# Zhongxu-Wang/ArtSpeech

Measured on AMD Instinct MI355X. Metric: mel frames/sec (whole job; per-GPU = value / n_gpus), acoustic-model inference path, batch 32 x 200-frame utterances, higher is better.
Workload: dtype f32 (f16x3 split-operand MFMA, fp32 accumulate)

## Files before the change

### artspeech_amd/csrc/common.h

```cpp
#pragma once
#include <hip/hip_runtime.h>
#include <stdint.h>

#define AS_OK 0
#define AS_EINVAL (-1)
#ifndef AS_EDEVICE
#define AS_EDEVICE (-3)
#endif

unsigned* as_status_words_device();
int as_status_peek();

#define AS_CHECK_LAUNCH()                        \
    do {                                         \
        hipError_t e__ = hipGetLastError();      \
        if (e__ != hipSuccess) return (int)e__;  \
    } while (0)

#define AS_CHECK(call)                           \
    do {                                         \
        hipError_t e__ = (call);                 \
        if (e__ != hipSuccess) return (int)e__;  \
    } while (0)

// ... 21 lines not shown
        if (r__ != AS_OK) return r__;                                              \
    } while (0)

#define AS_WAVE 64

struct AsDynGeo {
    const int32_t* frame_off;
    int32_t B, cap1, n_seg;
    int32_t seg_first[17];
    int32_t seg_cap[16];
    int32_t* seg_frame_off[16];
    int32_t* w[4];
    int32_t* off[4];
    unsigned long long* meta[4];
    int32_t* nvalid[4];
    int32_t* src3;
    int32_t* tof;
    unsigned* status;
};
int as_dyn_geometry_launch(const AsDynGeo& g, hipStream_t stream);
struct AsSegScatter {
    const float* src; int32_t ld_src, rows, n_seg;
    const int32_t* frame_off;
    int32_t seg_first[17];
    int32_t seg_cap[16];
    float* dst[16]; int32_t ld_dst[16];
};
int as_seg_scatter_launch(const AsSegScatter& a, hipStream_t stream);
int as_voice_gather_launch(const float* voices, int ld_voice, int n_voices, const int32_t* idx, int B, int n_style, int n_dur, float* style,
                           int ld_style, float* ds, int ld_ds, hipStream_t stream);
int as_durations_prosody_launch(const float* dur_f32, const int32_t* forced_dur, const int32_t* tok_off, int B, const float* pros, int ld_pros,
                                int32_t* dur_i32, int32_t* frame_off, int32_t* tok_of_frame, int max_frames, hipStream_t stream);
int as_project_cols_prosody_launch(const float* x, int ldx, int K, int N, const float* w, const float* bias, int M, float* y, int ldy,
                                   const float* pros, int ld_pros, const int32_t* col_off, int B, int track0, hipStream_t s);
int as_token_dur_scale_launch(const float* dur_f32, const float* rows, int ld, const int32_t* tok_off, int B, int ntok, const float* pros,
                              int ld_pros, float* out, hipStream_t stream);
int as_token_starts_launch(const int32_t* dur_i32, int ntok, int32_t* start, hipStream_t stream);
int as_token_tracks_launch(float* fne, int ld, int n_cols, const int32_t* tof, int n_frames_max, const int32_t* frame_off, const int32_t* tok_off,
                           int B, int ntok, const int32_t* start, const float* rows, int ld_rows, int smooth, hipStream_t stream);

int as_pcm16_launch(const float* w, int N, const int32_t* n_valid, float* w_fill, int16_t* pcm, hipStream_t stream);

#define AS_VOC_MAX_RATES 9
struct AsVocGeo {
    const int32_t* off;
    int32_t B, mult, cap, max_len, n_rates;
    int32_t rate[AS_VOC_MAX_RATES];
    long long meta_start[AS_VOC_MAX_RATES];
    int32_t* tab;
    unsigned long long* meta;
    int32_t* sample_off;
    unsigned* status;
};
int as_vocoder_cap_geometry_launch(const AsVocGeo& g, hipStream_t stream);

enum { AS_CLS_GEMM = 0, AS_CLS_ADAIN = 1, AS_CLS_LN = 2, AS_CLS_ATTN = 3, AS_CLS_LSTM = 4, AS_CLS_MAS = 5, AS_CLS_OTHER = 6, AS_N_CLS = 7 };
struct AsProfScope {
    int idx;
    hipStream_t stream;
    AsProfScope(int cls, double flops, double bytes, hipStream_t s, const char* tag = nullptr);
    ~AsProfScope();
};

#ifdef __HIPCC__
static __device__ __forceinline__ void as_status_raise(unsigned* words, int kind)
{
    if (words) __hip_atomic_store(words + kind, 1u, __ATOMIC_RELAXED, __HIP_MEMORY_SCOPE_SYSTEM);
}
static __device__ __forceinline__ int as_pcm16(float w, bool* nan)
{
    *nan = w != w;
    return *nan ? 0 : (int)fmaxf(-32768.f, fminf(32767.f, rintf(__fmul_rn(32767.f, w))));
}
static __device__ __forceinline__ float as_adain_val(float x, float mean, float rstd, float one_plus_gamma, float beta, int lrelu)
{
    const float o = __fmaf_rn(one_plus_gamma, __fmul_rn(__fsub_rn(x, mean), rstd), beta);
    return (lrelu && o < 0.f) ? __fmul_rn(0.2f, o) : o;
}
static __device__ __forceinline__ void as_convt_pair(float a0, float a1, float w0, float w1, float w2, float pb, float* o0, float* o1)
{
    *o0 = __fmaf_rn(a0, w1, pb);
    *o1 = __fadd_rn(__fmaf_rn(a1, w0, __fmul_rn(a0, w2)), pb);
}
#endif
```

### artspeech_amd/csrc/conv_gemm_h3.hip

```cpp
#include "conv_gemm.h"
#include <cstring>
#include <type_traits>

typedef __attribute__((address_space(3))) void lds_void;

template <int I, int N, typename F>
static __device__ __forceinline__ void h3_for(F&& f)
{
    if constexpr (I < N) {
        f(std::integral_constant<int, I>{});
        h3_for<I + 1, N>(f);
    }
}

template <int WM, int WN, int WK, int KT, int NS, int NP, int TM = 2>
struct H3Cfg {
    static constexpr int QP = NP == 1 ? 2 : 4;
    static constexpr int BM = 32 * TM * WM, BN = 64 * WN;
    static constexpr int KBS = WK * KT;
    static constexpr int A_BLK = QP * BM * 16, B_BLK = QP * BN * 16;
    static constexpr int A_ST = KBS * A_BLK;
    static constexpr int STAGE = KBS * (A_BLK + B_BLK);
    static constexpr int RED = (WK - 1) * WM * WN * 32 * TM * 64 * 4;
    static constexpr int LDS = NS * STAGE > RED ? NS * STAGE : RED;
// ... 407 lines not shown
{
    if ((double)K * ldx * 4.0 >= 2147483648.0) return AS_EINVAL;
    hipLaunchKernelGGL(split_f16x2_kernel, dim3(as_cdiv(N + 1, 1024), 2 * as_kbx(K)), dim3(256), 0, stream, x, ldx, K, N, n_valid, lrelu, slope,
                       reinterpret_cast<u32x4_t*>(xh));
    AS_CHECK_LAUNCH();
    return AS_OK;
}

extern "C" int as_split_f16x2_f32(const float* x, int ldx, int K, int N, int in_act, float in_slope, uint16_t* xh, as_stream_t stream)
{
    return as_split_f16x2_cap_f32(x, ldx, K, N, nullptr, in_act, in_slope, xh, stream);
}

extern "C" int as_split_f16x2_cap_f32(const float* x, int ldx, int K, int N, const int32_t* n_valid, int in_act, float in_slope, uint16_t* xh,
                                      as_stream_t stream)
{
    if (!x || !xh || K <= 0 || N < 0 || ldx < N || (in_act != 0 && in_act != 2) || !(fabsf(in_slope) <= 3.0e38f)) return AS_EINVAL;
    if ((reinterpret_cast<uintptr_t>(xh) & 15) != 0) return AS_EINVAL;
    if (N == 0) return AS_OK;
    AsProfScope prof__(AS_CLS_OTHER, 0, 8.0 * K * (double)N, (hipStream_t)stream);
    return as_split_f16x2_launch(x, ldx, K, N, in_act == 2, in_slope, xh, (hipStream_t)stream, n_valid);
}

extern "C" size_t as_prep_weight_f16x2_sc_bytes(int G, int Cout, int Cin, int T, int Cin2)
{
    if (G <= 0 || Cout <= 0 || Cin <= 0 || T <= 0 || Cin2 < 0) return 0;
    return (size_t)G * ((size_t)T * as_kbx(Cin) + (Cin2 ? as_kbx(Cin2) : 0)) * 4 * (size_t)Cout * 16;
}
extern "C" size_t as_prep_weight_f16x2_bytes(int G, int Cout, int Cin, int T) { return as_prep_weight_f16x2_sc_bytes(G, Cout, Cin, T, 0); }

extern "C" int as_prep_weight_f16x2_sc_host(const float* w, const float* w2, int G, int Cout, int Cin, int T, int Cin2, uint16_t* wh,
                                            float* scale_out)
{
    if (!w || !wh || !scale_out || G <= 0 || Cout <= 0 || Cin <= 0 || T <= 0 || Cin2 < 0 || ((Cin2 > 0) != (w2 != nullptr))) return AS_EINVAL;
    const size_t n = (size_t)G * Cout * Cin * T, n2 = (size_t)G * Cout * Cin2;
    float mx = 0.f;
    for (size_t i = 0; i < n + n2; ++i) {
        const float x = i < n ? w[i] : w2[i - n];
        const float v = x < 0 ? -x : x;
        if (!(v <= 3.0e38f)) return AS_EINVAL;
        mx = v > mx ? v : mx;
    }
    int e = 0;
    float scale = 1.0f;
    if (mx > 0.f) {
        frexpf(mx, &e);
        scale = ldexpf(1.0f, 14 - e);
    }
    const int KBx = as_kbx(Cin), KBx2 = Cin2 ? as_kbx(Cin2) : 0;
    const size_t blocks = (size_t)T * KBx + KBx2;
    const size_t total = as_prep_weight_f16x2_sc_bytes(G, Cout, Cin, T, Cin2) / 2;
    for (size_t i = 0; i < total; ++i) wh[i] = 0;
    auto put = [&](size_t block, int k, int m, float x) {
        const _Float16 h = (_Float16)x;
        const _Float16 l = (_Float16)(x - (float)h);
        const int kh = (k >> 3) & 1, e8 = k & 7;
        const size_t base = block * 4 * (size_t)Cout * 8;
        uint16_t hb, lb;
        __builtin_memcpy(&hb, &h, 2);
        __builtin_memcpy(&lb, &l, 2);
        wh[base + ((size_t)(0 * 2 + kh) * Cout + m) * 8 + e8] = hb;
        wh[base + ((size_t)(1 * 2 + kh) * Cout + m) * 8 + e8] = lb;
    };
    for (int g = 0; g < G; ++g)
        for (int m = 0; m < Cout; ++m) {
            for (int k = 0; k < Cin; ++k)
                for (int t = 0; t < T; ++t) put((size_t)g * blocks + (size_t)t * KBx + (k >> 4), k, m, w[(((size_t)g * Cout + m) * Cin + k) * T + t] * scale);
            for (int k = 0; k < Cin2; ++k) put((size_t)g * blocks + (size_t)T * KBx + (k >> 4), k, m, w2[((size_t)g * Cout + m) * Cin2 + k] * scale);
        }
    *scale_out = scale;
    return AS_OK;
}
extern "C" int as_prep_weight_f16x2_host(const float* w, int G, int Cout, int Cin, int T, uint16_t* wh, float* scale_out)
{
    return as_prep_weight_f16x2_sc_host(w, nullptr, G, Cout, Cin, T, 0, wh, scale_out);
}

static __device__ __forceinline__ float h3_wave_sum(float v)
{
#pragma unroll
    for (int o = 32; o > 0; o >>= 1) v += __shfl_xor(v, o);
    return v;
}

template <bool UP>
__global__ void __launch_bounds__(256)
adain_image_kernel(const AsAdainArgs a)
{
    const int lane = threadIdx.x & 63, wave = __builtin_amdgcn_readfirstlane(threadIdx.x >> 6);
    const int kb = blockIdx.x * 2 + (wave >> 1), kh = wave & 1, u = blockIdx.y;
    const int C = a.C;
    if (kb >= as_kbx(C)) return;
    const size_t NX = (size_t)a.N + 1;
    u32x4_t* xs = reinterpret_cast<u32x4_t*>(a.yh);
    const size_t plane = ((size_t)kb * 4 + kh) * NX;
    if (u == 0 && lane == 0) {
        xs[plane + a.N] = u32x4_t{0u, 0u, 0u, 0u};
        xs[plane + 2 * NX + a.N] = u32x4_t{0u, 0u, 0u, 0u};
    }
    const int o0 = a.col_off[u], L = a.col_w ? a.col_w[u] : a.col_off[u + 1] - o0;
    if (L <= 0) return;
    const int s0 = a.src_off ? a.src_off[u] : o0;
    const size_t gbase = a.gb_off ? (size_t)a.gb_off[u] : (size_t)u * a.ldgb;
    const int c0 = kb * 16 + kh * 8;
    float g1[8], bt[8], w0[8], w1[8], w2[8], pb[8];
#pragma unroll
    for (int r = 0; r < 8; ++r) {
        const int c = c0 + r < C ? c0 + r : C - 1;
        g1[r] = 1.0f + a.gb[gbase + (size_t)c * a.gb_sc];
        bt[r] = a.gb[gbase + (size_t)(C + c) * a.gb_sc];
        if (UP) { w0[r] = a.pool_w[c * 3 + 0]; w1[r] = a.pool_w[c * 3 + 1]; w2[r] = a.pool_w[c * 3 + 2]; pb[r] = a.pool_b[c]; }
    }
    const float* xr0 = a.x + s0;
    const size_t at0 = plane + (UP ? 2 * (size_t)o0 : (size_t)o0);
    float mean[8], rstd[8];
    auto resident = [&](auto rv_) {
        constexpr int RV = decltype(rv_)::value;
        float v[8][RV];
#pragma unroll
        for (int r = 0; r < 8; ++r) {
            const float* xr = xr0 + (size_t)(c0 + r < C ? c0 + r : C - 1) * a.ldx;
#pragma unroll
            for (int j = 0; j < RV; ++j) v[r][j] = xr[min(lane + 64 * j, L - 1)];
        }
#pragma unroll
        for (int r = 0; r < 8; ++r) {
            float sacc = 0.f;
#pragma unroll
            for (int j = 0; j < RV; ++j)
                if (lane + 64 * j < L) sacc += v[r][j];
            mean[r] = h3_wave_sum(sacc) / (float)L;
        }
#pragma unroll
        for (int r = 0; r < 8; ++r) {
            float vacc = 0.f;
#pragma unroll
            for (int j = 0; j < RV; ++j)
                if (lane + 64 * j < L) { const float d = __fsub_rn(v[r][j], mean[r]); vacc = __fmaf_rn(d, d, vacc); }
            rstd[r] = 1.0f / sqrtf(h3_wave_sum(vacc) / (float)L + 1e-5f);
        }
        if (UP && a.x_up) {
#pragma unroll
            for (int r = 0; r < 8; ++r) {
                if (c0 + r >= C) continue;
                float* ur = a.x_up + (size_t)(c0 + r) * a.ld_up + 2 * o0;
#pragma unroll
                for (int j = 0; j < RV; ++j) {
                    const int i = lane + 64 * j;
                    if (i < L) { ur[2 * i] = v[r][j]; ur[2 * i + 1] = v[r][j]; }
                }
            }
        }
#pragma unroll
        for (int r = 0; r < 8; ++r)
#pragma unroll
            for (int j = 0; j < RV; ++j)
                v[r][j] = (c0 + r < C && lane + 64 * j < L) ? as_adain_val(v[r][j], mean[r], rstd[r], g1[r], bt[r], a.lrelu) : 0.f;
#pragma unroll
        for (int j = 0; j < RV; ++j) {
            const int i = lane + 64 * j;
            if (64 * j >= L) break;
            if (!UP) {
                float t[8];
#pragma unroll
                for (int r = 0; r < 8; ++r) t[r] = v[r][j];
                u32x4_t h, l;
                split2(t, h, l);
                if (i < L) {
                    xs[at0 + i] = h;
                    xs[at0 + i + 2 * NX] = l;
                }
            } else {
                float e0[8], e1[8];
#pragma unroll
                for (int r = 0; r < 8; ++r) {
                    const float dn = __shfl_down(v[r][j], 1);
                    const float wr = j + 1 < RV ? __shfl(v[r][j + 1 < RV ? j + 1 : j], 0) : 0.f;
                    const float an = i + 1 < L ? (lane == 63 ? wr : dn) : 0.f;
                    float o0v, o1v;
                    as_convt_pair(v[r][j], an, w0[r], w1[r], w2[r], pb[r], &o0v, &o1v);
                    e0[r] = c0 + r < C ? o0v : 0.f;
                    e1[r] = c0 + r < C ? o1v : 0.f;
                }
                u32x4_t h, l, h2, l2;
                split2(e0, h, l);
                split2(e1, h2, l2);
                if (i < L) {
                    xs[at0 + 2 * i] = h;
                    xs[at0 + 2 * i + 2 * NX] = l;
                    xs[at0 + 2 * i + 1] = h2;
                    xs[at0 + 2 * i + 1 + 2 * NX] = l2;
                }
            }
        }
    };
    if (L <= 256) { resident(std::integral_constant<int, 4>{}); return; }
    if (L <= 512) { resident(std::integral_constant<int, 8>{}); return; }
    {
        size_t rowoff[8];
#pragma unroll
        for (int r = 0; r < 8; ++r) rowoff[r] = (size_t)(c0 + r < C ? c0 + r : C - 1) * a.ldx;
        float acc[8];
#pragma unroll
        for (int r = 0; r < 8; ++r) acc[r] = 0.f;
        int i = lane;
        for (; i + 192 < L; i += 256) {
            float t[4][8];
#pragma unroll
            for (int q = 0; q < 4; ++q)
#pragma unroll
                for (int r = 0; r < 8; ++r) t[q][r] = xr0[rowoff[r] + i + 64 * q];
#pragma unroll
            for (int q = 0; q < 4; ++q)
#pragma unroll
                for (int r = 0; r < 8; ++r) acc[r] += t[q][r];
        }
        for (; i < L; i += 64)
#pragma unroll
            for (int r = 0; r < 8; ++r) acc[r] += xr0[rowoff[r] + i];
#pragma unroll
        for (int r = 0; r < 8; ++r) { mean[r] = h3_wave_sum(acc[r]) / (float)L; acc[r] = 0.f; }
        i = lane;
        for (; i + 192 < L; i += 256) {
            float t[4][8];
#pragma unroll
            for (int q = 0; q < 4; ++q)
#pragma unroll
                for (int r = 0; r < 8; ++r) t[q][r] = xr0[rowoff[r] + i + 64 * q];
#pragma unroll
            for (int q = 0; q < 4; ++q)
#pragma unroll
                for (int r = 0; r < 8; ++r) { const float d = __fsub_rn(t[q][r], mean[r]); acc[r] = __fmaf_rn(d, d, acc[r]); }
        }
        for (; i < L; i += 64)
#pragma unroll
            for (int r = 0; r < 8; ++r) { const float d = __fsub_rn(xr0[rowoff[r] + i], mean[r]); acc[r] = __fmaf_rn(d, d, acc[r]); }
#pragma unroll
        for (int r = 0; r < 8; ++r) rstd[r] = 1.0f / sqrtf(h3_wave_sum(acc[r]) / (float)L + 1e-5f);
    }
    for (int i0 = lane; i0 < L; i0 += 128) {
        float xi[2][8], xn[2][8];
#pragma unroll
        for (int q = 0; q < 2; ++q) {
            const int i = min(i0 + 64 * q, L - 1);
#pragma unroll
            for (int r = 0; r < 8; ++r) {
                const float* xr = xr0 + (size_t)(c0 + r < C ? c0 + r : C - 1) * a.ldx;
                xi[q][r] = xr[i];
                if (UP) xn[q][r] = xr[min(i + 1, L - 1)];
            }
        }
#pragma unroll
        for (int q = 0; q < 2; ++q) {
            const int i = i0 + 64 * q;
            if (i >= L) break;
            float a0[8], a1[8];
#pragma unroll
            for (int r = 0; r < 8; ++r) {
                const bool ok = c0 + r < C;
                a0[r] = ok ? as_adain_val(xi[q][r], mean[r], rstd[r], g1[r], bt[r], a.lrelu) : 0.f;
                a1[r] = (UP && ok && i + 1 < L) ? as_adain_val(xn[q][r], mean[r], rstd[r], g1[r], bt[r], a.lrelu) : 0.f;
                if (UP && a.x_up && ok) {
                    float* ur = a.x_up + (size_t)(c0 + r) * a.ld_up + 2 * o0 + 2 * i;
                    ur[0] = xi[q][r];
                    ur[1] = xi[q][r];
                }
            }
            u32x4_t h, l;
            if (!UP) {
                split2(a0, h, l);
                xs[at0 + i] = h;
                xs[at0 + i + 2 * NX] = l;
            } else {
                float e0[8], e1[8];
#pragma unroll
                for (int r = 0; r < 8; ++r) {
                    as_convt_pair(a0[r], a1[r], w0[r], w1[r], w2[r], pb[r], &e0[r], &e1[r]);
                    if (c0 + r >= C) { e0[r] = 0.f; e1[r] = 0.f; }
                }
                split2(e0, h, l);
                xs[at0 + 2 * i] = h;
                xs[at0 + 2 * i + 2 * NX] = l;
                split2(e1, h, l);
                xs[at0 + 2 * i + 1] = h;
                xs[at0 + 2 * i + 1 + 2 * NX] = l;
            }
        }
    }
}

extern "C" int as_adain_image_f32(const AsAdainArgs* args_host, as_stream_t stream)
{
    if (!args_host) return AS_EINVAL;
    const AsAdainArgs& a = *args_host;
    if (!a.x || !a.gb || !a.col_off || !a.yh || a.C <= 0 || a.U <= 0 || a.N < 0 || a.gb_sc <= 0 || (!a.gb_off && a.ldgb <= 0)) return AS_EINVAL;
    if ((a.pool_w == nullptr) != (a.pool_b == nullptr) || (a.x_up && !a.pool_w)) return AS_EINVAL;
    if ((reinterpret_cast<uintptr_t>(a.yh) & 15) != 0) return AS_EINVAL;
    if (a.N == 0) return AS_OK;
    AsProfScope prof__(AS_CLS_ADAIN, 0, 8.0 * a.C * (double)a.N, (hipStream_t)stream);
    if (a.pool_w) hipLaunchKernelGGL(adain_image_kernel<true>, dim3(as_kbx(a.C) / 2, a.U), dim3(256), 0, (hipStream_t)stream, a);
    else hipLaunchKernelGGL(adain_image_kernel<false>, dim3(as_kbx(a.C) / 2, a.U), dim3(256), 0, (hipStream_t)stream, a);
    AS_CHECK_LAUNCH();
    return AS_OK;
}

extern "C" int as_adain_split_f32(const float* x, int ldx, int C, const float* gamma_beta, int ldgb, const int32_t* col_off, int B,
                                  int N, int lrelu, uint16_t* xs, as_stream_t stream)
{
    if (!x || !gamma_beta || !col_off || !xs || C <= 0 || B <= 0 || N < 0 || ldgb < 2 * C) return AS_EINVAL;
    AsAdainArgs a = {};
    a.x = x; a.ldx = ldx; a.C = C; a.gb = gamma_beta; a.ldgb = ldgb; a.gb_sc = 1; a.col_off = col_off; a.U = B; a.N = N; a.lrelu = lrelu; a.yh = xs;
    return as_adain_image_f32(&a, stream);
}

__global__ void __launch_bounds__(256)
rows_image_kernel(const float* __restrict__ x, int ldx, int K, int B, u32x4_t* __restrict__ xh)
{
    const int i = blockIdx.x * 256 + threadIdx.x;
    const int groups = 2 * as_kbx(K);
    if (i >= groups * (B + 1)) return;
    const int g = i / (B + 1), b = i % (B + 1);
    float t[8];
#pragma unroll
    for (int r = 0; r < 8; ++r) t[r] = (b < B && g * 8 + r < K) ? x[(size_t)b * ldx + g * 8 + r] : 0.f;
    u32x4_t h, l;
    split2(t, h, l);
    const size_t at = ((size_t)(g >> 1) * 4 + (g & 1)) * (B + 1) + b;
    xh[at] = h;
    xh[at + 2 * (size_t)(B + 1)] = l;
}

extern "C" int as_rows_image_f32(const float* x, int ldx, int K, int B, uint16_t* xh, as_stream_t stream)
{
    if (!x || !xh || K <= 0 || B <= 0 || ldx < K || (reinterpret_cast<uintptr_t>(xh) & 15) != 0) return AS_EINVAL;
    AsProfScope prof__(AS_CLS_OTHER, 0, 8.0 * K * (double)B, (hipStream_t)stream);
    hipLaunchKernelGGL(rows_image_kernel, dim3(as_cdiv((long)2 * as_kbx(K) * (B + 1), 256)), dim3(256), 0, (hipStream_t)stream, x, ldx, K, B,
                       reinterpret_cast<u32x4_t*>(xh));
    AS_CHECK_LAUNCH();
    return AS_OK;
}

#define LNS_COLS 32
#define LNS_PARTS 32
#define LNS_MAXG 4
__global__ void __launch_bounds__(1024)
channel_ln_split_kernel(const float* __restrict__ x, int ldx, int C, int N, const float* __restrict__ gamma1,
                        const float* __restrict__ beta1, const float* __restrict__ gamma2, const float* __restrict__ beta2, int n_split,
                        float eps, int relu, u32x4_t* __restrict__ xs, int KBx)
{
    __shared__ float red[LNS_PARTS][LNS_COLS + 1];
    const int col = threadIdx.x % LNS_COLS, part = threadIdx.x / LNS_COLS;
    const int j = blockIdx.x * LNS_COLS + col;
    const bool ok = j < N;
    const int grp = gamma2 ? j / n_split : 0;
    const float* gamma = gamma1 + (ptrdiff_t)grp * (gamma2 - gamma1);
    const float* beta = beta1 + (ptrdiff_t)grp * (beta2 - beta1);
    const int ngroups = 2 * KBx;
    float v[LNS_MAXG][8];
    float s = 0.f;
#pragma unroll
    for (int i = 0; i < LNS_MAXG; ++i)
#pragma unroll
        for (int r = 0; r < 8; ++r) {
            const int c = 8 * (part + i * LNS_PARTS) + r;
            v[i][r] = (ok && c < C) ? x[(size_t)c * ldx + j] : 0.f;
            s += v[i][r];
        }
    red[part][col] = s;
    __syncthreads();
    float tot = 0.f;
#pragma unroll
    for (int q = 0; q < LNS_PARTS; ++q) tot += red[q][col];
    const float mean = tot / (float)C;
    __syncthreads();
    float q2 = 0.f;
#pragma unroll
    for (int i = 0; i < LNS_MAXG; ++i)
#pragma unroll
        for (int r = 0; r < 8; ++r) {
            const int c = 8 * (part + i * LNS_PARTS) + r;
            const float d = __fsub_rn(v[i][r], mean);
            if (c < C) q2 = __fmaf_rn(d, d, q2);
        }
    red[part][col] = q2;
    __syncthreads();
    tot = 0.f;
#pragma unroll
    for (int q = 0; q < LNS_PARTS; ++q) tot += red[q][col];
    const float rs = 1.0f / sqrtf(tot / (float)C + eps);
    const size_t NX = (size_t)N + 1;
    if (blockIdx.x == 0 && col == 0) {
#pragma unroll
        for (int i = 0; i < LNS_MAXG; ++i) {
            const int g = part + i * LNS_PARTS;
            if (g < ngroups)
                for (int p = 0; p < 2; ++p) xs[((size_t)(g >> 1) * 4 + (g & 1) + 2 * p) * NX + N] = u32x4_t{0u, 0u, 0u, 0u};
        }
    }
    if (!ok) return;
#pragma unroll
    for (int i = 0; i < LNS_MAXG; ++i) {
        const int g = part + i * LNS_PARTS;
        if (g >= ngroups) continue;
        float t[8];
#pragma unroll
        for (int r = 0; r < 8; ++r) {
            const int c = 8 * g + r;
            float o = 0.f;
            if (c < C) {
                o = __fmaf_rn(__fmul_rn(__fsub_rn(v[i][r], mean), rs), gamma[c], beta[c]);
                if (relu) o = o < 0.f ? 0.f : o;
            }
            t[r] = o;
        }
        u32x4_t h, l;
        split2(t, h, l);
        const size_t at = ((size_t)(g >> 1) * 4 + (g & 1)) * NX + j;
        xs[at] = h;
        xs[at + 2 * NX] = l;
    }
}

extern "C" int as_channel_layernorm_split_f32(const float* x, int ldx, int C, int N, const float* gamma, const float* beta,
                                              const float* gamma2, const float* beta2, int n_split, float eps, int relu, uint16_t* xs,
                                              as_stream_t stream)
{
    if (!x || !xs || !gamma || !beta || C <= 0 || C > 8 * LNS_PARTS * LNS_MAXG || N <= 0 || ldx < N ||
        ((gamma2 == nullptr) != (beta2 == nullptr)) || (gamma2 && n_split <= 0) || (reinterpret_cast<uintptr_t>(xs) & 15) != 0)
        return AS_EINVAL;
    const int KBx = as_kbx(C);
    AsProfScope prof__(AS_CLS_LN, 8.0 * C * N, 8.0 * C * (double)N, (hipStream_t)stream);
    hipLaunchKernelGGL(channel_ln_split_kernel, dim3(as_cdiv(N, LNS_COLS)), dim3(1024), 0, (hipStream_t)stream, x, ldx, C, N, gamma, beta,
                       gamma2, beta2, n_split, eps, relu, reinterpret_cast<u32x4_t*>(xs), KBx);
    AS_CHECK_LAUNCH();
    return AS_OK;
}
```

### artspeech_amd/csrc/elementwise.hip

```cpp
#include "common.h"
#include <algorithm>
#include <cstring>
#include "artspeech_hip.h"
#include "conv_gemm.h"
#include "down_strips.h"
#include <cstdint>
#include <type_traits>
#define AS_FILE_CLS AS_CLS_OTHER

static __device__ __forceinline__ float wave_sum(float v)
{
#pragma unroll
    for (int o = 32; o > 0; o >>= 1) v += __shfl_xor(v, o);
    return v;
}

static __device__ __forceinline__ float lrelu02(float v) { return v > 0.f ? v : 0.2f * v; }

__global__ void make_meta_kernel(const int* __restrict__ widths, const int* __restrict__ col_off, int B, int H,
                                 unsigned long long* __restrict__ meta, unsigned* __restrict__ status)
{
    const int b = blockIdx.y;
    const int W = widths[b];
    const int base = col_off[b];
// ... 136 lines not shown

extern "C" int as_channel_layernorm_f32(const float* x, int ldx, int C, int N, const float* gamma, const float* beta,
                                        float eps, int relu, float* y, int ldy, as_stream_t stream)
{
    return as_channel_layernorm_groups_f32(x, ldx, C, N, gamma, beta, nullptr, nullptr, 0, eps, relu, y, ldy, stream);
}

__global__ void __launch_bounds__(256)
adain_kernel(const float* __restrict__ x, int ldx, int C, const float* __restrict__ gb, int ldgb,
             const int* __restrict__ col_off, int B, float* __restrict__ y, int ldy, int act,
             const float* __restrict__ pool_w, const float* __restrict__ pool_b, float* __restrict__ xup, int ldup)
{
    const int lane = threadIdx.x & 63;
    const int row = blockIdx.x * 4 + (threadIdx.x >> 6);
    if (row >= C * B) return;
    const int c = row / B, b = row - c * B;
    const int o0 = col_off[b], L = col_off[b + 1] - o0;
    if (L <= 0) return;
    const float* xr = x + (size_t)c * ldx + o0;
    float s = 0.f;
    for (int i = lane; i < L; i += 64) s += xr[i];
    const float mean = wave_sum(s) / (float)L;
    float v = 0.f;
    for (int i = lane; i < L; i += 64) { const float d = __fsub_rn(xr[i], mean); v = __fmaf_rn(d, d, v); }
    const float var = wave_sum(v) / (float)L;
    const float rs = 1.0f / sqrtf(var + 1e-5f);
    const float g = 1.0f + gb[(size_t)b * ldgb + c];
    const float be = gb[(size_t)b * ldgb + C + c];
    if (!pool_w) {
        float* yr = y + (size_t)c * ldy + o0;
        for (int i = lane; i < L; i += 64) yr[i] = as_adain_val(xr[i], mean, rs, g, be, act);
    } else {
        const float w0 = pool_w[c * 3 + 0], w1 = pool_w[c * 3 + 1], w2 = pool_w[c * 3 + 2], pb = pool_b[c];
        float* yr = y + (size_t)c * ldy + 2 * o0;
        float* ur = xup ? xup + (size_t)c * ldup + 2 * o0 : nullptr;
        for (int i = lane; i < L; i += 64) {
            const float xi = xr[i];
            const float a0 = as_adain_val(xi, mean, rs, g, be, act);
            const float a1 = i + 1 < L ? as_adain_val(xr[i + 1], mean, rs, g, be, act) : 0.f;
            float e0, e1;
            as_convt_pair(a0, a1, w0, w1, w2, pb, &e0, &e1);
            yr[2 * i] = e0;
            yr[2 * i + 1] = e1;
            if (ur) { ur[2 * i] = xi; ur[2 * i + 1] = xi; }
        }
    }
}

extern "C" int as_adain_f32(const float* x, int ldx, int C, const float* gamma_beta, int ldgb, const int32_t* col_off,
                            int B, float* y, int ldy, int lrelu, const float* pool_w, const float* pool_b,
                            float* x_up, int ld_up, as_stream_t stream)
{
    if (!x || !y || !gamma_beta || !col_off || C <= 0 || B < 0 || ldgb < 2 * C) return AS_EINVAL;
    if ((pool_w == nullptr) != (pool_b == nullptr)) return AS_EINVAL;
    if (B == 0) return AS_OK;
    AsProfScope prof__(AS_CLS_ADAIN, 0, 0, (hipStream_t)stream);
    hipLaunchKernelGGL(adain_kernel, dim3(as_cdiv((long)C * B, 4)), dim3(256), 0, (hipStream_t)stream, x, ldx, C,
                       gamma_beta, ldgb, col_off, B, y, ldy, lrelu, pool_w, pool_b, x_up, ld_up);
    AS_CHECK_LAUNCH();
    return AS_OK;
}

template <int KR>
__global__ void __launch_bounds__(256)
linear_rows_kernel(const float* __restrict__ x, int ldx, const float* __restrict__ w, const float* __restrict__ bias,
                   int B, int M, int K, float* __restrict__ y, int ldy)
{
    static_assert(KR == 1 || KR == 2 || KR == 4 || KR == 8, "quads of the weight row per lane");
    const int lane = threadIdx.x & 63;
    const int m = blockIdx.x * 4 + (threadIdx.x >> 6);
    if (m >= M) return;
    const float* wr = w + (size_t)m * K;
    const float bm = bias ? bias[m] : 0.f;
    const bool vec = (K & 3) == 0 && (ldx & 3) == 0 && ((reinterpret_cast<uintptr_t>(w) | reinterpret_cast<uintptr_t>(x)) & 15) == 0;
    if (vec && K <= 256 * KR) {
        constexpr int RT = 32 / KR;
        const int nq = K >> 2;
        float4 wq[KR];
#pragma unroll
        for (int c = 0; c < KR; ++c) {
            const int q = lane + 64 * c;
            wq[c] = q < nq ? reinterpret_cast<const float4*>(wr)[q] : make_float4(0.f, 0.f, 0.f, 0.f);
        }
        for (int b0 = 0; b0 < B; b0 += RT) {
            float4 v[RT][KR];
#pragma unroll
            for (int r = 0; r < RT; ++r) {
                const float4* xq = reinterpret_cast<const float4*>(x + (size_t)min(b0 + r, B - 1) * ldx);
#pragma unroll
                for (int c = 0; c < KR; ++c) {
                    const int q = lane + 64 * c;
                    v[r][c] = xq[q < nq ? q : 0];
                }
            }
#pragma unroll
            for (int r = 0; r < RT; ++r) {
                float s = 0.f;
#pragma unroll
                for (int c = 0; c < KR; ++c) s += wq[c].x * v[r][c].x + wq[c].y * v[r][c].y + wq[c].z * v[r][c].z + wq[c].w * v[r][c].w;
                s = wave_sum(s);
                if (lane == 0 && b0 + r < B) y[(size_t)(b0 + r) * ldy + m] = s + bm;
            }
        }
        return;
    }
    for (int b = 0; b < B; ++b) {
        const float* xr = x + (size_t)b * ldx;
        float s = 0.f;
        for (int k = lane; k < K; k += 64) s += wr[k] * xr[k];
        s = wave_sum(s);
        if (lane == 0) y[(size_t)b * ldy + m] = s + bm;
    }
}

extern "C" int as_linear_rows_f32(const float* x, int ldx, const float* w, const float* bias, int B, int M, int K,
                                  float* y, int ldy, as_stream_t stream)
{
    if (!x || !w || !y || B < 0 || M <= 0 || K <= 0 || ldx < K || ldy < M) return AS_EINVAL;
    if (B == 0) return AS_OK;
    AsProfScope prof__(AS_FILE_CLS, 0, 0, (hipStream_t)stream);
    const dim3 grid(as_cdiv(M, 4)), block(256);
    hipStream_t s_ = (hipStream_t)stream;
    if (K <= 256) hipLaunchKernelGGL(linear_rows_kernel<1>, grid, block, 0, s_, x, ldx, w, bias, B, M, K, y, ldy);
    else if (K <= 512) hipLaunchKernelGGL(linear_rows_kernel<2>, grid, block, 0, s_, x, ldx, w, bias, B, M, K, y, ldy);
    else if (K <= 1024) hipLaunchKernelGGL(linear_rows_kernel<4>, grid, block, 0, s_, x, ldx, w, bias, B, M, K, y, ldy);
    else hipLaunchKernelGGL(linear_rows_kernel<8>, grid, block, 0, s_, x, ldx, w, bias, B, M, K, y, ldy);
    AS_CHECK_LAUNCH();
    return AS_OK;
}

template <int MM>
__global__ void __launch_bounds__(256)
project_cols_kernel(const float* __restrict__ x, int ldx, int K, int N, const float* w, const float* __restrict__ bias, int M,
                    float* __restrict__ y, int ldy, const float* __restrict__ pros, int ldr, const int* __restrict__ col_off, int B, int track0)
{
    __shared__ float part[3][MM][64];
    extern __shared__ __attribute__((aligned(16))) float wsm[];
    for (int i = threadIdx.x; i < MM * K; i += 256) {
        const int k = i / MM, m = i % MM;
        wsm[i] = m < M ? w[(size_t)m * K + k] : 0.f;
    }
    __syncthreads();
    w = wsm;
    const int lane = threadIdx.x & 63, wave = threadIdx.x >> 6;
    const int j = blockIdx.x * 64 + lane;
    const bool ok = j < N;
    float acc[MM];
#pragma unroll
    for (int m = 0; m < MM; ++m) acc[m] = 0.f;
    int k = wave;
    const float* xc = x + (ok ? j : 0);
    for (; k + 60 < K; k += 64) {
        float v[16];
#pragma unroll
        for (int u = 0; u < 16; ++u) v[u] = xc[(size_t)(k + 4 * u) * ldx];
#pragma unroll
        for (int u = 0; u < 16; ++u)
#pragma unroll
            for (int m = 0; m < MM; ++m)
                acc[m] += w[(k + 4 * u) * MM + m] * v[u];
    }
    for (; k + 12 < K; k += 16) {
        float v[4];
#pragma unroll
        for (int u = 0; u < 4; ++u) v[u] = xc[(size_t)(k + 4 * u) * ldx];
#pragma unroll
        for (int u = 0; u < 4; ++u)
#pragma unroll
            for (int m = 0; m < MM; ++m)
                acc[m] += w[(k + 4 * u) * MM + m] * v[u];
    }
    for (; k < K; k += 4) {
        const float v = xc[(size_t)k * ldx];
#pragma unroll
        for (int m = 0; m < MM; ++m)
            acc[m] += w[k * MM + m] * v;
    }
    if (wave > 0) {
#pragma unroll
        for (int m = 0; m < MM; ++m) part[wave - 1][m][lane] = acc[m];
    }
    __syncthreads();
    if (wave != 0 || !ok) return;
    const float* r = nullptr;
    if (pros) {
        int lo = 0, hi = B;
        while (hi > lo) {
            const int mid = (lo + hi + 1) >> 1;
            if (col_off[mid] <= j) lo = mid;
            else hi = mid - 1;
        }
        if (lo < B) r = pros + (size_t)lo * ldr + track0;
    }
#pragma unroll
    for (int m = 0; m < MM; ++m) {
        if (m >= M) continue;
        const float v = ((acc[m] + part[0][m][lane]) + (part[1][m][lane] + part[2][m][lane])) + (bias ? bias[m] : 0.f);
        y[(size_t)m * ldy + j] = r ? __builtin_fmaf(r[AS_PROSODY_GAIN + m], v, r[AS_PROSODY_OFFSET + m]) : v;
    }
}

extern "C" int as_project_cols_f32(const float* x, int ldx, int K, int N, const float* w, const float* bias, int M, float* y, int ldy,
                                   as_stream_t stream)
{
// ... 1043 lines not shown
```

Measured before the change: 1.785 million.

## Batch wave reductions and vectorize loads in AdaIN, channel LN and linear-rows kernels

Adds an 8-way batched wave reduction built on ds_bpermute and uses it in the AdaIN image kernel and the linear-rows kernel, so independent per-row sums share one LDS wait per step instead of each running its own shuffle chain. AdaIN now loads its per-utterance offsets with one lane-parallel load and broadcasts them with readlane, gathers gamma/beta/pool weights across lanes, and writes upsample pairs as float2. Channel LN is templated on the group count so registers and loops match C, and it loads the affine parameters early with float4 reads. Linear-rows gets a second grid dimension over batch rows so small-M launches fill more of the GPU. The inline asm and the wider templating add register pressure and code-size risk.

```diff
diff --git a/artspeech_amd/csrc/common.h b/artspeech_amd/csrc/common.h
--- a/artspeech_amd/csrc/common.h
+++ b/artspeech_amd/csrc/common.h
@@ -127,4 +127,25 @@
     *o0 = __fmaf_rn(a0, w1, pb);
     *o1 = __fadd_rn(__fmaf_rn(a1, w0, __fmul_rn(a0, w2)), pb);
 }
+static __device__ __forceinline__ void as_wave_sum8(float (&s)[8])
+{
+    const int lane = __lane_id();
+#pragma unroll
+    for (int o = 32; o > 0; o >>= 1) {
+        const int at = (lane ^ o) << 2;
+        float t0, t1, t2, t3, t4, t5, t6, t7;
+        asm volatile("ds_bpermute_b32 %0, %8, %9\n\t"
+                     "ds_bpermute_b32 %1, %8, %10\n\t"
+                     "ds_bpermute_b32 %2, %8, %11\n\t"
+                     "ds_bpermute_b32 %3, %8, %12\n\t"
+                     "ds_bpermute_b32 %4, %8, %13\n\t"
+                     "ds_bpermute_b32 %5, %8, %14\n\t"
+                     "ds_bpermute_b32 %6, %8, %15\n\t"
+                     "ds_bpermute_b32 %7, %8, %16\n\t"
+                     "s_waitcnt lgkmcnt(0)"
+                     : "=&v"(t0), "=&v"(t1), "=&v"(t2), "=&v"(t3), "=&v"(t4), "=&v"(t5), "=&v"(t6), "=&v"(t7)
+                     : "v"(at), "v"(s[0]), "v"(s[1]), "v"(s[2]), "v"(s[3]), "v"(s[4]), "v"(s[5]), "v"(s[6]), "v"(s[7]));
+        s[0] += t0; s[1] += t1; s[2] += t2; s[3] += t3; s[4] += t4; s[5] += t5; s[6] += t6; s[7] += t7;
+    }
+}
 #endif
diff --git a/artspeech_amd/csrc/conv_gemm_h3.hip b/artspeech_amd/csrc/conv_gemm_h3.hip
--- a/artspeech_amd/csrc/conv_gemm_h3.hip
+++ b/artspeech_amd/csrc/conv_gemm_h3.hip
@@ -513,7 +513,6 @@
     for (int o = 32; o > 0; o >>= 1) v += __shfl_xor(v, o);
     return v;
 }
-
 template <bool UP>
 __global__ void __launch_bounds__(256)
 adain_image_kernel(const AsAdainArgs a)
@@ -522,28 +521,65 @@
     const int kb = blockIdx.x * 2 + (wave >> 1), kh = wave & 1, u = blockIdx.y;
     const int C = a.C;
     if (kb >= as_kbx(C)) return;
+    const int32_t* __restrict__ col_off = a.col_off;
+    const int32_t* __restrict__ col_w = a.col_w;
+    const int32_t* __restrict__ src_off = a.src_off;
+    const int32_t* __restrict__ gb_off = a.gb_off;
+    const float* __restrict__ gb = a.gb;
+    const float* __restrict__ pool_w = a.pool_w;
+    const float* __restrict__ pool_b = a.pool_b;
+    int word = 0;
+    {
+        const int32_t* p = col_off + u;
+        if (lane == 1 && !col_w) p = col_off + u + 1;
+        if (lane == 2 && col_w) p = col_w + u;
+        if (lane == 3 && src_off) p = src_off + u;
+        if (lane == 4 && gb_off) p = gb_off + u;
+        if (lane < 5) word = *p;
+    }
+    const int o0 = __builtin_amdgcn_readlane(word, 0);
+    const int L = col_w ? __builtin_amdgcn_readlane(word, 2) : __builtin_amdgcn_readlane(word, 1) - o0;
+    const int s0 = src_off ? __builtin_amdgcn_readlane(word, 3) : o0;
+    const size_t gbase = gb_off ? (size_t)__builtin_amdgcn_readlane(word, 4) : (size_t)u * a.ldgb;
     const size_t NX = (size_t)a.N + 1;
     u32x4_t* xs = reinterpret_cast<u32x4_t*>(a.yh);
     const size_t plane = ((size_t)kb * 4 + kh) * NX;
-    if (u == 0 && lane == 0) {
-        xs[plane + a.N] = u32x4_t{0u, 0u, 0u, 0u};
-        xs[plane + 2 * NX + a.N] = u32x4_t{0u, 0u, 0u, 0u};
-    }
-    const int o0 = a.col_off[u], L = a.col_w ? a.col_w[u] : a.col_off[u + 1] - o0;
-    if (L <= 0) return;
-    const int s0 = a.src_off ? a.src_off[u] : o0;
-    const size_t gbase = a.gb_off ? (size_t)a.gb_off[u] : (size_t)u * a.ldgb;
+    auto zero_column = [&]() {
+        if (u == 0 && lane == 0) {
+            xs[plane + a.N] = u32x4_t{0u, 0u, 0u, 0u};
+            xs[plane + 2 * NX + a.N] = u32x4_t{0u, 0u, 0u, 0u};
+        }
+    };
+    if (L <= 0) { zero_column(); return; }
     const int c0 = kb * 16 + kh * 8;
     float g1[8], bt[8], w0[8], w1[8], w2[8], pb[8];
-#pragma unroll
-    for (int r = 0; r < 8; ++r) {
+    float gb_l, pw_l = 0.f, pb_l = 0.f;
+    {
+        const int r = lane & 7;
         const int c = c0 + r < C ? c0 + r : C - 1;
-        g1[r] = 1.0f + a.gb[gbase + (size_t)c * a.gb_sc];
-        bt[r] = a.gb[gbase + (size_t)(C + c) * a.gb_sc];
-        if (UP) { w0[r] = a.pool_w[c * 3 + 0]; w1[r] = a.pool_w[c * 3 + 1]; w2[r] = a.pool_w[c * 3 + 2]; pb[r] = a.pool_b[c]; }
-    }
+        gb_l = gb[gbase + (size_t)((lane & 8) ? C + c : c) * a.gb_sc];
+        if (UP) {
+            const int rw = min(lane / 3, 7), cw = c0 + rw < C ? c0 + rw : C - 1;
+            pw_l = pool_w[cw * 3 + (lane - 3 * (lane / 3))];
+            pb_l = pool_b[c];
+        }
+    }
+    auto constants = [&]() {
+#pragma unroll
+        for (int r = 0; r < 8; ++r) {
+            g1[r] = 1.0f + __builtin_bit_cast(float, __builtin_amdgcn_readlane(__builtin_bit_cast(int, gb_l), r));
+            bt[r] = __builtin_bit_cast(float, __builtin_amdgcn_readlane(__builtin_bit_cast(int, gb_l), 8 + r));
+            if (UP) {
+                w0[r] = __builtin_bit_cast(float, __builtin_amdgcn_readlane(__builtin_bit_cast(int, pw_l), 3 * r + 0));
+                w1[r] = __builtin_bit_cast(float, __builtin_amdgcn_readlane(__builtin_bit_cast(int, pw_l), 3 * r + 1));
+                w2[r] = __builtin_bit_cast(float, __builtin_amdgcn_readlane(__builtin_bit_cast(int, pw_l), 3 * r + 2));
+                pb[r] = __builtin_bit_cast(float, __builtin_amdgcn_readlane(__builtin_bit_cast(int, pb_l), r));
+            }
+        }
+    };
     const float* xr0 = a.x + s0;
     const size_t at0 = plane + (UP ? 2 * (size_t)o0 : (size_t)o0);
+    const bool up_pair = UP && (reinterpret_cast<uintptr_t>(a.x_up) & 7) == 0 && (a.ld_up & 1) == 0;
     float mean[8], rstd[8];
     auto resident = [&](auto rv_) {
         constexpr int RV = decltype(rv_)::value;
@@ -560,16 +596,24 @@
 #pragma unroll
             for (int j = 0; j < RV; ++j)
                 if (lane + 64 * j < L) sacc += v[r][j];
-            mean[r] = h3_wave_sum(sacc) / (float)L;
-        }
+            mean[r] = sacc;
+        }
+        as_wave_sum8(mean);
+#pragma unroll
+        for (int r = 0; r < 8; ++r) mean[r] = mean[r] / (float)L;
 #pragma unroll
         for (int r = 0; r < 8; ++r) {
             float vacc = 0.f;
 #pragma unroll
             for (int j = 0; j < RV; ++j)
                 if (lane + 64 * j < L) { const float d = __fsub_rn(v[r][j], mean[r]); vacc = __fmaf_rn(d, d, vacc); }
-            rstd[r] = 1.0f / sqrtf(h3_wave_sum(vacc) / (float)L + 1e-5f);
-        }
+            rstd[r] = vacc;
+        }
+        as_wave_sum8(rstd);
+#pragma unroll
+        for (int r = 0; r < 8; ++r) rstd[r] = 1.0f / sqrtf(rstd[r] / (float)L + 1e-5f);
+        constants();
+        zero_column();
         if (UP && a.x_up) {
 #pragma unroll
             for (int r = 0; r < 8; ++r) {
@@ -578,7 +622,9 @@
 #pragma unroll
                 for (int j = 0; j < RV; ++j) {
                     const int i = lane + 64 * j;
-                    if (i < L) { ur[2 * i] = v[r][j]; ur[2 * i + 1] = v[r][j]; }
+                    if (i >= L) continue;
+                    if (up_pair) *reinterpret_cast<float2*>(ur + 2 * i) = make_float2(v[r][j], v[r][j]);
+                    else { ur[2 * i] = v[r][j]; ur[2 * i + 1] = v[r][j]; }
                 }
             }
         }
@@ -602,12 +648,15 @@
                     xs[at0 + i + 2 * NX] = l;
                 }
             } else {
-                float e0[8], e1[8];
+                float e0[8], e1[8], dn[8], wr[8];
 #pragma unroll
                 for (int r = 0; r < 8; ++r) {
-                    const float dn = __shfl_down(v[r][j], 1);
-                    const float wr = j + 1 < RV ? __shfl(v[r][j + 1 < RV ? j + 1 : j], 0) : 0.f;
-                    const float an = i + 1 < L ? (lane == 63 ? wr : dn) : 0.f;
+                    dn[r] = __shfl_down(v[r][j], 1);
+                    wr[r] = j + 1 < RV ? __shfl(v[r][j + 1 < RV ? j + 1 : j], 0) : 0.f;
+                }
+#pragma unroll
+                for (int r = 0; r < 8; ++r) {
+                    const float an = i + 1 < L ? (lane == 63 ? wr[r] : dn[r]) : 0.f;
                     float o0v, o1v;
                     as_convt_pair(v[r][j], an, w0[r], w1[r], w2[r], pb[r], &o0v, &o1v);
                     e0[r] = c0 + r < C ? o0v : 0.f;
@@ -646,11 +695,16 @@
 #pragma unroll
                 for (int r = 0; r < 8; ++r) acc[r] += t[q][r];
         }
-        for (; i < L; i += 64)
-#pragma unroll
-            for (int r = 0; r < 8; ++r) acc[r] += xr0[rowoff[r] + i];
-#pragma unroll
-        for (int r = 0; r < 8; ++r) { mean[r] = h3_wave_sum(acc[r]) / (float)L; acc[r] = 0.f; }
+        for (; i < L; i += 64) {
+            float t[8];
+#pragma unroll
+            for (int r = 0; r < 8; ++r) t[r] = xr0[rowoff[r] + i];
+#pragma unroll
+            for (int r = 0; r < 8; ++r) acc[r] += t[r];
+        }
+        as_wave_sum8(acc);
+#pragma unroll
+        for (int r = 0; r < 8; ++r) { mean[r] = acc[r] / (float)L; acc[r] = 0.f; }
         i = lane;
         for (; i + 192 < L; i += 256) {
             float t[4][8];
@@ -663,12 +717,19 @@
 #pragma unroll
                 for (int r = 0; r < 8; ++r) { const float d = __fsub_rn(t[q][r], mean[r]); acc[r] = __fmaf_rn(d, d, acc[r]); }
         }
-        for (; i < L; i += 64)
-#pragma unroll
-            for (int r = 0; r < 8; ++r) { const float d = __fsub_rn(xr0[rowoff[r] + i], mean[r]); acc[r] = __fmaf_rn(d, d, acc[r]); }
-#pragma unroll
-        for (int r = 0; r < 8; ++r) rstd[r] = 1.0f / sqrtf(h3_wave_sum(acc[r]) / (float)L + 1e-5f);
-    }
+        for (; i < L; i += 64) {
+            float t[8];
+#pragma unroll
+            for (int r = 0; r < 8; ++r) t[r] = xr0[rowoff[r] + i];
+#pragma unroll
+            for (int r = 0; r < 8; ++r) { const float d = __fsub_rn(t[r], mean[r]); acc[r] = __fmaf_rn(d, d, acc[r]); }
+        }
+        as_wave_sum8(acc);
+#pragma unroll
+        for (int r = 0; r < 8; ++r) rstd[r] = 1.0f / sqrtf(acc[r] / (float)L + 1e-5f);
+    }
+    constants();
+    zero_column();
     for (int i0 = lane; i0 < L; i0 += 128) {
         float xi[2][8], xn[2][8];
 #pragma unroll
@@ -693,8 +754,8 @@
                 a1[r] = (UP && ok && i + 1 < L) ? as_adain_val(xn[q][r], mean[r], rstd[r], g1[r], bt[r], a.lrelu) : 0.f;
                 if (UP && a.x_up && ok) {
                     float* ur = a.x_up + (size_t)(c0 + r) * a.ld_up + 2 * o0 + 2 * i;
-                    ur[0] = xi[q][r];
-                    ur[1] = xi[q][r];
+                    if (up_pair) *reinterpret_cast<float2*>(ur) = make_float2(xi[q][r], xi[q][r]);
+                    else { ur[0] = xi[q][r]; ur[1] = xi[q][r]; }
                 }
             }
             u32x4_t h, l;
@@ -774,6 +835,7 @@
 #define LNS_COLS 32
 #define LNS_PARTS 32
 #define LNS_MAXG 4
+template <int NG, bool QUADS>
 __global__ void __launch_bounds__(1024)
 channel_ln_split_kernel(const float* __restrict__ x, int ldx, int C, int N, const float* __restrict__ gamma1,
                         const float* __restrict__ beta1, const float* __restrict__ gamma2, const float* __restrict__ beta2, int n_split,
@@ -783,20 +845,49 @@
     const int col = threadIdx.x % LNS_COLS, part = threadIdx.x / LNS_COLS;
     const int j = blockIdx.x * LNS_COLS + col;
     const bool ok = j < N;
-    const int grp = gamma2 ? j / n_split : 0;
+    const int grp = (gamma2 && ok) ? j / n_split : 0;
     const float* gamma = gamma1 + (ptrdiff_t)grp * (gamma2 - gamma1);
     const float* beta = beta1 + (ptrdiff_t)grp * (beta2 - beta1);
     const int ngroups = 2 * KBx;
-    float v[LNS_MAXG][8];
-    float s = 0.f;
-#pragma unroll
-    for (int i = 0; i < LNS_MAXG; ++i)
+    float v[NG][8];
+#pragma unroll
+    for (int i = 0; i < NG; ++i)
 #pragma unroll
         for (int r = 0; r < 8; ++r) {
             const int c = 8 * (part + i * LNS_PARTS) + r;
             v[i][r] = (ok && c < C) ? x[(size_t)c * ldx + j] : 0.f;
-            s += v[i][r];
-        }
+        }
+    float gq[NG][8], bq[NG][8];
+    auto load_affine = [&]() {
+        if (QUADS) {
+            const int last = (C >> 2) - 1;
+    #pragma unroll
+            for (int i = 0; i < NG; ++i)
+    #pragma unroll
+                for (int h = 0; h < 2; ++h) {
+                    const int q = min(2 * (part + i * LNS_PARTS) + h, last);
+                    const float4 gv = reinterpret_cast<const float4*>(gamma)[q], bv = reinterpret_cast<const float4*>(beta)[q];
+                    gq[i][4 * h + 0] = gv.x; gq[i][4 * h + 1] = gv.y; gq[i][4 * h + 2] = gv.z; gq[i][4 * h + 3] = gv.w;
+                    bq[i][4 * h + 0] = bv.x; bq[i][4 * h + 1] = bv.y; bq[i][4 * h + 2] = bv.z; bq[i][4 * h + 3] = bv.w;
+                }
+        } else {
+    #pragma unroll
+            for (int i = 0; i < NG; ++i)
+    #pragma unroll
+                for (int r = 0; r < 8; ++r) {
+                    const int c = min(8 * (part + i * LNS_PARTS) + r, C - 1);
+                    gq[i][r] = gamma[c];
+                    bq[i][r] = beta[c];
+                }
+        }
+    };
+    constexpr bool EARLY = NG <= 2;
+    if (EARLY) load_affine();
+    float s = 0.f;
+#pragma unroll
+    for (int i = 0; i < NG; ++i)
+#pragma unroll
+        for (int r = 0; r < 8; ++r) s += v[i][r];
     red[part][col] = s;
     __syncthreads();
     float tot = 0.f;
@@ -806,7 +897,7 @@
     __syncthreads();
     float q2 = 0.f;
 #pragma unroll
-    for (int i = 0; i < LNS_MAXG; ++i)
+    for (int i = 0; i < NG; ++i)
 #pragma unroll
         for (int r = 0; r < 8; ++r) {
             const int c = 8 * (part + i * LNS_PARTS) + r;
@@ -822,7 +913,7 @@
     const size_t NX = (size_t)N + 1;
     if (blockIdx.x == 0 && col == 0) {
 #pragma unroll
-        for (int i = 0; i < LNS_MAXG; ++i) {
+        for (int i = 0; i < NG; ++i) {
             const int g = part + i * LNS_PARTS;
             if (g < ngroups)
                 for (int p = 0; p < 2; ++p) xs[((size_t)(g >> 1) * 4 + (g & 1) + 2 * p) * NX + N] = u32x4_t{0u, 0u, 0u, 0u};
@@ -830,7 +921,7 @@
     }
     if (!ok) return;
 #pragma unroll
-    for (int i = 0; i < LNS_MAXG; ++i) {
+    for (int i = 0; i < NG; ++i) {
         const int g = part + i * LNS_PARTS;
         if (g >= ngroups) continue;
         float t[8];
@@ -839,7 +930,7 @@
             const int c = 8 * g + r;
             float o = 0.f;
             if (c < C) {
-                o = __fmaf_rn(__fmul_rn(__fsub_rn(v[i][r], mean), rs), gamma[c], beta[c]);
+                o = __fmaf_rn(__fmul_rn(__fsub_rn(v[i][r], mean), rs), EARLY ? gq[i][r] : gamma[c], EARLY ? bq[i][r] : beta[c]);
                 if (relu) o = o < 0.f ? 0.f : o;
             }
             t[r] = o;
@@ -861,8 +952,16 @@
         return AS_EINVAL;
     const int KBx = as_kbx(C);
     AsProfScope prof__(AS_CLS_LN, 8.0 * C * N, 8.0 * C * (double)N, (hipStream_t)stream);
-    hipLaunchKernelGGL(channel_ln_split_kernel, dim3(as_cdiv(N, LNS_COLS)), dim3(1024), 0, (hipStream_t)stream, x, ldx, C, N, gamma, beta,
-                       gamma2, beta2, n_split, eps, relu, reinterpret_cast<u32x4_t*>(xs), KBx);
+    const dim3 grid(as_cdiv(N, LNS_COLS)), block(1024);
+    u32x4_t* im = reinterpret_cast<u32x4_t*>(xs);
+    const bool quads = (C & 3) == 0 && ((reinterpret_cast<uintptr_t>(gamma) | reinterpret_cast<uintptr_t>(beta) | reinterpret_cast<uintptr_t>(gamma2) |
+                                         reinterpret_cast<uintptr_t>(beta2)) & 15) == 0;
+    auto launch = [&](auto kernel) {
+        hipLaunchKernelGGL(kernel, grid, block, 0, (hipStream_t)stream, x, ldx, C, N, gamma, beta, gamma2, beta2, n_split, eps, relu, im, KBx);
+    };
+    if (C <= 256) quads ? launch(channel_ln_split_kernel<1, true>) : launch(channel_ln_split_kernel<1, false>);
+    else if (C <= 512) quads ? launch(channel_ln_split_kernel<2, true>) : launch(channel_ln_split_kernel<2, false>);
+    else launch(channel_ln_split_kernel<LNS_MAXG, false>);
     AS_CHECK_LAUNCH();
     return AS_OK;
 }
diff --git a/artspeech_amd/csrc/elementwise.hip b/artspeech_amd/csrc/elementwise.hip
--- a/artspeech_amd/csrc/elementwise.hip
+++ b/artspeech_amd/csrc/elementwise.hip
@@ -242,7 +242,7 @@
             const int q = lane + 64 * c;
             wq[c] = q < nq ? reinterpret_cast<const float4*>(wr)[q] : make_float4(0.f, 0.f, 0.f, 0.f);
         }
-        for (int b0 = 0; b0 < B; b0 += RT) {
+        for (int b0 = blockIdx.y * RT; b0 < B; b0 += RT * gridDim.y) {
             float4 v[RT][KR];
 #pragma unroll
             for (int r = 0; r < RT; ++r) {
@@ -253,24 +253,35 @@
                     v[r][c] = xq[q < nq ? q : 0];
                 }
             }
+            float s[RT];
 #pragma unroll
             for (int r = 0; r < RT; ++r) {
-                float s = 0.f;
-#pragma unroll
-                for (int c = 0; c < KR; ++c) s += wq[c].x * v[r][c].x + wq[c].y * v[r][c].y + wq[c].z * v[r][c].z + wq[c].w * v[r][c].w;
-                s = wave_sum(s);
-                if (lane == 0 && b0 + r < B) y[(size_t)(b0 + r) * ldy + m] = s + bm;
+                s[r] = 0.f;
+#pragma unroll
+                for (int c = 0; c < KR; ++c) s[r] += wq[c].x * v[r][c].x + wq[c].y * v[r][c].y + wq[c].z * v[r][c].z + wq[c].w * v[r][c].w;
             }
+            if constexpr (RT >= 8) {
+#pragma unroll
+                for (int r = 0; r < RT; r += 8) as_wave_sum8(*reinterpret_cast<float(*)[8]>(&s[r]));
+            } else {
+#pragma unroll
+                for (int r = 0; r < RT; ++r) s[r] = wave_sum(s[r]);
+            }
+#pragma unroll
+            for (int r = 0; r < RT; ++r)
+                if (lane == 0 && b0 + r < B) y[(size_t)(b0 + r) * ldy + m] = s[r] + bm;
         }
         return;
     }
-    for (int b = 0; b < B; ++b) {
-        const float* xr = x + (size_t)b * ldx;
-        float s = 0.f;
-        for (int k = lane; k < K; k += 64) s += wr[k] * xr[k];
-        s = wave_sum(s);
-        if (lane == 0) y[(size_t)b * ldy + m] = s + bm;
-    }
+    constexpr int RT = 32 / KR;
+    for (int b0 = blockIdx.y * RT; b0 < B; b0 += RT * gridDim.y)
+        for (int b = b0; b < min(b0 + RT, B); ++b) {
+            const float* xr = x + (size_t)b * ldx;
+            float s = 0.f;
+            for (int k = lane; k < K; k += 64) s += wr[k] * xr[k];
+            s = wave_sum(s);
+            if (lane == 0) y[(size_t)b * ldy + m] = s + bm;
+        }
 }
 
 extern "C" int as_linear_rows_f32(const float* x, int ldx, const float* w, const float* bias, int B, int M, int K,
@@ -279,7 +290,9 @@
     if (!x || !w || !y || B < 0 || M <= 0 || K <= 0 || ldx < K || ldy < M) return AS_EINVAL;
     if (B == 0) return AS_OK;
     AsProfScope prof__(AS_FILE_CLS, 0, 0, (hipStream_t)stream);
-    const dim3 grid(as_cdiv(M, 4)), block(256);
+    const int gx = as_cdiv(M, 4), rt = K <= 256 ? 32 : K <= 512 ? 16 : K <= 1024 ? 8 : 4;
+    const int gy = gx < 256 ? std::min(as_cdiv(B, rt), as_cdiv(256, gx)) : 1;
+    const dim3 grid(gx, gy), block(256);
     hipStream_t s_ = (hipStream_t)stream;
     if (K <= 256) hipLaunchKernelGGL(linear_rows_kernel<1>, grid, block, 0, s_, x, ldx, w, bias, B, M, K, y, ldy);
     else if (K <= 512) hipLaunchKernelGGL(linear_rows_kernel<2>, grid, block, 0, s_, x, ldx, w, bias, B, M, K, y, ldy);
```

New measurement: 1.781 million. No clear change (-0.2%).
